# Wang-Ruocheng/QuanONet

Hardware: AMD Instinct MI355X
Metric: train samples/sec (circuit-evals/sec alongside), QuanONet Q=5 Net40-2-20-2 Advection (higher is better)
Workload: dtype f64

## Files before the change

### quanonet_amd/csrc/hea_zyz.hpp

```cpp
#pragma once
#include "hea_device.hpp"
#include "hea_sincos.hpp"

namespace qhea {

constexpr int kRecBytes = 1024;
constexpr int kRecRy = 512;
constexpr int kZCsBytes = 20480;

__host__ __device__ inline long zyz_cs_row(int n, long E) { return E + 2 * n; }
__host__ __device__ inline bool zyz_eligible(int n, long E) {
    return n >= 2 && n <= 5 && (long)(64 >> n) * zyz_cs_row(n, E) * 16 <= kZCsBytes;
}
__host__ __device__ inline int zyz_layer_count(const Runs& r, int n) {
    long L = 0;
    for (int i = 0; i < r.nruns; ++i) L += (long)r.count[i] * ((r.enc[i] + n - 1) / n + r.ld[i]);
    return (int)L;
}

struct AngleSrc {
    const double* x;
    EncDesc enc;
    long m_rows = 0, m_params = 0;
};
// ... 7 lines not shown
    const int si = e < a.enc.seg[0].ncols ? 0 : 1;
    const EncSeg& sg = a.enc.seg[si];
    const int ee = si ? e - a.enc.seg[0].ncols : e;
    const long m = blockIdx.y;
    const double v = sg.in[(b + m * a.m_rows) * sg.width + ee % sg.width];
    const long ep = ee + m * a.m_params;
    return sg.w ? v * sg.w[ep] + sg.b[ep] : v * (MSCALE ? mscale : sg.scale);
}
__device__ __forceinline__ double enc_angle(const AngleSrc& a, int E, long b, int e) { return enc_angle_impl<false>(a, E, b, e, 0.0); }
__device__ __forceinline__ double enc_angle(const AngleSrcM& a, int E, long b, int e) { return enc_angle_impl<true>(a.s, E, b, e, a.scale); }
template <class S>
__device__ __forceinline__ void fill_cs(double2* cs, const S& src, int n, int E, long b0, long B, int ns, int tid, int nthreads,
                                        int row_stride = 0 ) {
    const int row = row_stride ? row_stride : (int)zyz_cs_row(n, E);
    for (int i = tid; i < ns * E; i += nthreads) {
        const int s = i / E, e = i - s * E;
        const long b = (b0 + s < B) ? b0 + s : B - 1;
        double sn, cn;
        fast_sincos(0.5 * enc_angle(src, E, b, e), &sn, &cn);
        cs[s * row + n + e] = make_double2(cn, sn);
    }
}

template <int Q>
__device__ __forceinline__ unsigned lane_sign_mask(int lane) { return ((unsigned)lane << (31 - Q)) & 0x80000000u; }
__device__ __forceinline__ double flip_sign(double v, unsigned mask) {
    return __hiloint2double(__double2hiint(v) ^ (int)mask, __double2loint(v));
}

template <bool DAGGER>
__device__ __forceinline__ void apply_phase(double& re, double& im, const double2& d) {
    const double s = DAGGER ? -d.y : d.y;
    const double nr = d.x * re - s * im;
    im = d.x * im + s * re;
    re = nr;
}
template <int Q, bool DAGGER>
__device__ __forceinline__ void apply_ry(double& re, double& im, const double2& u) {
    const double sv = DAGGER ? -u.y : u.y;
    if constexpr (Q == 4) {
        const auto lo = __builtin_amdgcn_permlane16_swap((unsigned)__double2loint(re), (unsigned)__double2loint(im), false, false);
        const auto hi = __builtin_amdgcn_permlane16_swap((unsigned)__double2hiint(re), (unsigned)__double2hiint(im), false, false);
        const double a = __hiloint2double((int)hi[0], (int)lo[0]), b = __hiloint2double((int)hi[1], (int)lo[1]);
        const double o1 = u.x * a - sv * b, o2 = sv * a + u.x * b;
        const auto l2 = __builtin_amdgcn_permlane16_swap((unsigned)__double2loint(o1), (unsigned)__double2loint(o2), false, false);
        const auto h2 = __builtin_amdgcn_permlane16_swap((unsigned)__double2hiint(o1), (unsigned)__double2hiint(o2), false, false);
        re = __hiloint2double((int)h2[0], (int)l2[0]);
        im = __hiloint2double((int)h2[1], (int)l2[1]);
    } else {
        const double qr = xchg<(1 << Q)>(re), qi = xchg<(1 << Q)>(im);
        re = u.x * re + sv * qr;
        im = u.x * im + sv * qi;
    }
}
template <int N, int Q, bool DAGGER>
__device__ __forceinline__ void apply_enc(double (&re)[1], double (&im)[1], const double2& cs) {
    if constexpr (Q == 4) apply_ry<4, DAGGER>(re[0], im[0], cs);
    else apply_rx<N, Q>(re, im, cs.x, DAGGER ? -cs.y : cs.y);
}

typedef unsigned int u32x4 __attribute__((ext_vector_type(4)));
__device__ __forceinline__ void dma_record(const u32x4& rsrc, unsigned lds_addr, unsigned voff, unsigned soff) {
    asm volatile("s_mov_b32 m0, %0\n\ts_nop 0\n\tbuffer_load_dwordx4 %1, %2, %3 offen lds"
                 :: "s"(lds_addr), "v"(voff), "s"(rsrc), "s"(soff) : "memory", "m0");
}
template <int NREC>
__device__ __forceinline__ void dma_records(const u32x4& rsrc, unsigned lds_addr, unsigned voff, unsigned soff) {
    static_assert(NREC >= 1 && NREC <= 3 && kRecBytes == 1024, "instruction offsets are 12 bits");
    if constexpr (NREC == 1)
        asm volatile("s_mov_b32 m0, %0\n\ts_nop 0\n\tbuffer_load_dwordx4 %1, %2, %3 offen lds"
                     :: "s"(lds_addr), "v"(voff), "s"(rsrc), "s"(soff) : "memory", "m0");
    else if constexpr (NREC == 2)
        asm volatile("s_mov_b32 m0, %0\n\ts_nop 0\n\tbuffer_load_dwordx4 %1, %2, %3 offen lds\n\t"
                     "buffer_load_dwordx4 %1, %2, %3 offen offset:1024 lds"
                     :: "s"(lds_addr), "v"(voff), "s"(rsrc), "s"(soff) : "memory", "m0");
    else
        asm volatile("s_mov_b32 m0, %0\n\ts_nop 0\n\tbuffer_load_dwordx4 %1, %2, %3 offen lds\n\t"
                     "buffer_load_dwordx4 %1, %2, %3 offen offset:1024 lds\n\t"
                     "buffer_load_dwordx4 %1, %2, %3 offen offset:2048 lds"
                     :: "s"(lds_addr), "v"(voff), "s"(rsrc), "s"(soff) : "memory", "m0");
}
template <int CNT>
__device__ __forceinline__ void wait_vmcnt() { asm volatile("s_waitcnt vmcnt(%0)" :: "n"(CNT) : "memory"); }

constexpr int kSlots = 8, kDist = 6;
#ifndef QHEA_ZSIGMA
#define QHEA_ZSIGMA 4
#endif
constexpr int kZSigma = QHEA_ZSIGMA;
constexpr int kAxisRing = 16;
#ifdef QHEA_PROFILE_WAITS
struct ZSync { int psi_prod, lam_prod, ready, abort; int cursor[4]; unsigned long long waited[24]; int next; };
#else
struct ZSync { int psi_prod, lam_prod, ready, abort; int cursor[kZSigma]; int next; };
#endif
constexpr int kRecRingBytes = kSlots * kRecBytes;

template <int N>
struct LayerStream {
    u32x4 rsrc;
    char* ring;
    unsigned lds0;
    unsigned lane16, dgoff;
    unsigned voff[N];
    int L;
    double2 dg;
    double2 ry[N];

    __device__ __forceinline__ void init(const char* table, int bytes, char* ring_wave, int lane, int klow, int nlayers) {
        const unsigned long long base = reinterpret_cast<unsigned long long>(table);
        rsrc = u32x4{(unsigned)base, (unsigned)(base >> 32) & 0xffffu, (unsigned)bytes, 0x00020000u};
        ring = ring_wave;
        lds0 = (unsigned)(unsigned long long)(__attribute__((address_space(3))) char*)ring_wave;
        lane16 = (unsigned)lane * 16u;
        dgoff = (unsigned)klow * 16u;
        L = nlayers;
        static_for<0, N>([&](auto q) {
            constexpr int Q = decltype(q)::value;
            voff[Q] = kRecRy + Q * 32 + (Q == 4 ? 1u : (((unsigned)lane >> Q) & 1u)) * 16u;
        });
    }
    __device__ __forceinline__ void issue(int l) const {
        const int lc = l < 0 ? 0 : (l > L ? L : l);
        dma_record(rsrc, lds0 + (unsigned)(l & (kSlots - 1)) * kRecBytes, lane16, (unsigned)lc * kRecBytes);
    }
    __device__ __forceinline__ char* buf(int l) const { return ring + (l & (kSlots - 1)) * kRecBytes; }
    __device__ __forceinline__ double2 rd_diag(int l) const { return *reinterpret_cast<const double2*>(buf(l) + dgoff); }
    template <int Q>
    __device__ __forceinline__ double2 rd_ry(int l) const { return *reinterpret_cast<const double2*>(buf(l) + voff[Q]); }
    __device__ __forceinline__ void rd_all_ry(int l) { static_for<0, N>([&](auto q) { ry[decltype(q)::value] = rd_ry<decltype(q)::value>(l); }); }

    template <int D>
    __device__ __forceinline__ void prime(int l0) {
#pragma unroll
        for (int i = 0; i < kDist; ++i) issue(l0 + i * D);
        wait_vmcnt<kDist - 1>();
        dg = rd_diag(l0);
        rd_all_ry(l0);
    }
    template <int D>
    __device__ __forceinline__ void begin(int l) {
        issue(l + kDist * D);
        wait_vmcnt<kDist - 1>();
    }
};

template <int N>
__device__ __forceinline__ void zyz_forward(double (&re)[1], double (&im)[1], const Runs& runs, LayerStream<N>& ls,
                                            const double2* __restrict__ csrow, int E, int lane, int klow, int ring_fwd) {
    re[0] = klow == 0 ? 1.0 : 0.0;
    im[0] = 0.0;
    int l = 0, col = 0;
    ls.template prime<1>(0);
    double2 nxt[N];
    auto prefetch = [&](int c) {
        static_for<0, N>([&](auto q) {
            constexpr int Q = decltype(q)::value;
            const int e = c + Q;
            nxt[Q] = csrow[e < E ? e : (E > 0 ? E - 1 : 0)];
        });
    };
    if (E > 0) prefetch(0);
    for (int ri = 0; ri < runs.nruns; ++ri) {
        const int ne = runs.enc[ri], nld = runs.ld[ri];
        for (int rep = 0; rep < runs.count[ri]; ++rep) {
            for (int j0 = 0; j0 < ne; j0 += N) {
                const int m = (ne - j0) < N ? (ne - j0) : N;
                ls.template begin<1>(l);
                apply_phase<false>(re[0], im[0], ls.dg);
                ls.dg = ls.rd_diag(l + 1);
                for_gates_below<N>(m, [&](auto q) {
                    constexpr int Q = decltype(q)::value;
                    apply_enc<N, Q, false>(re, im, nxt[Q]);
                });
                prefetch(col + j0 + m);
                ls.rd_all_ry(l + 1);
                ++l;
            }
            col += ne;
            for (int s = 0; s < nld; ++s) {
                ls.template begin<1>(l);
                apply_phase<false>(re[0], im[0], ls.dg);
                ls.dg = ls.rd_diag(l + 1);
                static_for<0, N>([&](auto q) {
                    constexpr int Q = decltype(q)::value;
                    apply_ry<Q, false>(re[0], im[0], ls.ry[Q]);
                    ls.ry[Q] = ls.template rd_ry<Q>(l + 1);
                });
                re[0] = lane_gather(re[0], ring_fwd);
                im[0] = lane_gather(im[0], ring_fwd);
                ++l;
            }
        }
    }
    apply_phase<false>(re[0], im[0], ls.dg);
}

template <int K> using CtSlot = std::integral_constant<int, K>;
struct RtSlot { int b; };
template <class T> struct is_ct_slot : std::false_type {};
template <int K> struct is_ct_slot<CtSlot<K>> : std::true_type {};
constexpr int kBSlots = 4, kBDist = 2;
constexpr int kPadRecs = 9;
constexpr int kBlockRingBytes = kBSlots * 3 * kRecBytes;

template <int N, int LD, bool SHARED = false>
struct BlockStream {
    static constexpr int RPB = 1 + LD;
    bool loader = true;
    u32x4 rsrc;
    char* ring;
    unsigned lds0, lane16, a_dg;
    unsigned a_ry[N];
    double2 dg[RPB];
    double2 ry[LD][N];
    double2 cs[N];

    __device__ __forceinline__ void init(const char* rec0, int nrec , char* ring_wave, int lane, int klow) {
        const unsigned long long base = reinterpret_cast<unsigned long long>(rec0) - (unsigned long long)kPadRecs * kRecBytes;
        rsrc = u32x4{(unsigned)base, (unsigned)(base >> 32) & 0xffffu, (unsigned)((nrec + 2 * kPadRecs) * kRecBytes), 0x00020000u};
        ring = ring_wave;
        lds0 = (unsigned)(unsigned long long)(__attribute__((address_space(3))) char*)ring_wave;
        lane16 = (unsigned)lane * 16u;
        a_dg = (unsigned)klow * 16u;
        static_for<0, N>([&](auto q) {
            constexpr int Q = decltype(q)::value;
            a_ry[Q] = kRecRy + Q * 32 + (Q == 4 ? 1u : (((unsigned)lane >> Q) & 1u)) * 16u;
        });
    }
    __device__ __forceinline__ void issue(int b) const {
        const unsigned slot = lds0 + (unsigned)(b & (kBSlots - 1)) * (RPB * kRecBytes);
        const unsigned soff = (unsigned)((b * RPB + kPadRecs) * kRecBytes);
        dma_records<RPB>(rsrc, slot, lane16, soff);
    }
    __device__ __forceinline__ const char* slot(int b) const { return ring + (b & (kBSlots - 1)) * (RPB * kRecBytes); }
    template <int D, int K>
    static constexpr int slot_off(CtSlot<K>) { return ((K + D) & (kBSlots - 1)) * (RPB * kRecBytes); }
    template <int D>
    static __device__ __forceinline__ int slot_off(RtSlot s) { return ((s.b + D) & (kBSlots - 1)) * (RPB * kRecBytes); }
    template <int D, class SL>
    __device__ __forceinline__ const char* slot_rel(SL s) const { return ring + slot_off<D>(s); }
    template <int D, class SL>
    __device__ __forceinline__ void ahead_rel(SL s, int b) const {
        if (!SHARED || loader)
            dma_records<RPB>(rsrc, lds0 + (unsigned)slot_off<D>(s), lane16, (unsigned)(((b + D) * RPB + kPadRecs) * kRecBytes));
    }
    __device__ __forceinline__ void landed() const {
        if (!SHARED || loader) wait_vmcnt<(kBDist - 1) * RPB>();
        if constexpr (SHARED) __syncthreads();
    }
    __device__ __forceinline__ void landed_late() const {
        if (!SHARED || loader) wait_vmcnt<kBDist * RPB>();
        if constexpr (SHARED) __syncthreads();
    }
    template <int D>
    __device__ __forceinline__ void ahead(int b) const { if (!SHARED || loader) issue(b + (kBDist + 1) * D); }
    template <int D>
    __device__ __forceinline__ void step(int b) const {
        ahead<D>(b);
        if (!SHARED || loader) wait_vmcnt<kBDist * RPB>();
        if constexpr (SHARED) __syncthreads();
    }
    template <int D>
    __device__ __forceinline__ void prime(int b0, bool drain) const {
        if (!SHARED || loader) {
            if (drain) wait_vmcnt<0>();
        }
        if constexpr (SHARED) { if (drain) __syncthreads(); }
        if (!SHARED || loader) {
#pragma unroll
            for (int i = 0; i <= kBDist; ++i) issue(b0 + i * D);
            wait_vmcnt<kBDist * RPB>();
        }
        if constexpr (SHARED) __syncthreads();
    }
    static __device__ __forceinline__ double2 rd(const char* p, unsigned off) { return *reinterpret_cast<const double2*>(p + off); }
    __device__ __forceinline__ void load_records(const char* sl) {
#pragma unroll
        for (int i = 0; i < RPB; ++i) dg[i] = rd(sl, i * kRecBytes + a_dg);
#pragma unroll
        for (int s = 0; s < LD; ++s)
            static_for<0, N>([&](auto q) { ry[s][decltype(q)::value] = rd(sl, (1 + s) * kRecBytes + a_ry[decltype(q)::value]); });
    }
    __device__ __forceinline__ void load_cs(const double2* __restrict__ csrow, int c0) {
        const double2* p = csrow + c0;
        static_for<0, N>([&](auto q) { cs[decltype(q)::value] = p[decltype(q)::value]; });
    }
};

__host__ __device__ inline int zyz_fast_ld(const Runs& r, int n) {
    if (r.nruns < 1) return 0;
    const int ld = r.ld[0];
    if (ld != 1 && ld != 2) return 0;
    for (int i = 0; i < r.nruns; ++i)
        if (r.ld[i] != ld || r.enc[i] != n || r.count[i] < 1) return 0;
    return ld;
}

template <int N>
struct LayerCoef { double2 dg; double2 g[N]; };

template <int N, int LD, class BS>
__device__ __forceinline__ void zyz_forward_fast(double (&re)[1], double (&im)[1], const Runs& runs, BS& bs,
                                                 const double2* __restrict__ csrow, int E, int lane, int klow, int ring_fwd) {
    re[0] = klow == 0 ? 1.0 : 0.0;
    im[0] = 0.0;
    bs.template prime<1>(0, false);
    int nblocks = 0;
    for (int ri = 0; ri < runs.nruns; ++ri) nblocks += runs.count[ri];
    const double2* cs_b = csrow;
    LayerCoef<N> ce, ca, cb;
    ce.dg = bs.rd(bs.slot(0), bs.a_dg);
    static_for<0, N>([&](auto q) { ce.g[decltype(q)::value] = cs_b[decltype(q)::value]; });
    auto read_layer = [&](LayerCoef<N>& c, const char* sl, int rec) {
        c.dg = bs.rd(sl, rec * kRecBytes + bs.a_dg);
        static_for<0, N>([&](auto q) { c.g[decltype(q)::value] = bs.rd(sl, rec * kRecBytes + bs.a_ry[decltype(q)::value]); });
        __builtin_amdgcn_sched_barrier(0);
    };
    auto read_chunk = [&](const char* nx, int kb) {
        ce.dg = bs.rd(nx, bs.a_dg);
        const double2* cn = cs_b + (kb + 1) * N;
        static_for<0, N>([&](auto q) { ce.g[decltype(q)::value] = cn[decltype(q)::value]; });
        __builtin_amdgcn_sched_barrier(0);
    };
    auto ry_layer = [&](const LayerCoef<N>& c) {
        apply_phase<false>(re[0], im[0], c.dg);
        static_for<0, N>([&](auto q) { apply_ry<decltype(q)::value, false>(re[0], im[0], c.g[decltype(q)::value]); });
        __builtin_amdgcn_sched_barrier(0);
        re[0] = lane_gather(re[0], ring_fwd);
        im[0] = lane_gather(im[0], ring_fwd);
    };
    auto block = [&](auto sl, int b, int kb) {
        const char* cur = bs.template slot_rel<0>(sl);
        const char* nx = bs.template slot_rel<1>(sl);
        read_layer(ca, cur, 1);
        apply_phase<false>(re[0], im[0], ce.dg);
        static_for<0, N>([&](auto q) { apply_enc<N, decltype(q)::value, false>(re, im, ce.g[decltype(q)::value]); });
        if constexpr (LD == 2) {
            read_layer(cb, cur, 2);
            ry_layer(ca);
            bs.template ahead_rel<kBDist + 1>(sl, b);
            __builtin_amdgcn_sched_barrier(0);
            bs.landed_late();
            read_chunk(nx, kb);
            ry_layer(cb);
        } else {
            bs.landed();
            read_chunk(nx, kb);
            ry_layer(ca);
            bs.template ahead_rel<kBDist + 1>(sl, b);
            __builtin_amdgcn_sched_barrier(0);
        }
    };
    int b = 0;
    for (; b + kBSlots <= nblocks; b += kBSlots) {
        block(CtSlot<0>{}, b, 0);
        block(CtSlot<1>{}, b + 1, 1);
        block(CtSlot<2>{}, b + 2, 2);
// ... 23 lines not shown
    }
}
template <int Q>
__device__ __forceinline__ double2 cs32_packed(const double2* chunk ) {
    if constexpr (Q == 4) { const double2 t = chunk[2 * Q]; return make_double2(t.y, t.x); }
    else return chunk[2 * Q + 1];
}

template <bool HALVES>
__device__ __forceinline__ void swap_dup(double x, double& A, double& B) {
    double y;
    asm("" : "=v"(y) : "0"(x));
    const unsigned lo = (unsigned)__double2loint(x), hi = (unsigned)__double2hiint(x);
    const unsigned lo2 = (unsigned)__double2loint(y), hi2 = (unsigned)__double2hiint(y);
    if constexpr (HALVES) {
        const auto l = __builtin_amdgcn_permlane32_swap(lo, lo2, false, false);
        const auto h = __builtin_amdgcn_permlane32_swap(hi, hi2, false, false);
        A = __hiloint2double((int)h[0], (int)l[0]); B = __hiloint2double((int)h[1], (int)l[1]);
    } else {
        const auto l = __builtin_amdgcn_permlane16_swap(lo, lo2, false, false);
        const auto h = __builtin_amdgcn_permlane16_swap(hi, hi2, false, false);
        A = __hiloint2double((int)h[0], (int)l[0]); B = __hiloint2double((int)h[1], (int)l[1]);
    }
}
__device__ __forceinline__ void split_phase(double& x, const double2& d ) {
    double A, B;
    swap_dup<true>(x, A, B);
    x = d.y * A + d.x * B;
}
template <int Q>
__device__ __forceinline__ void split_ry(double& x, const double2& u) {
    if constexpr (Q == 4) {
        double A, B;
        swap_dup<false>(x, A, B);
        x = u.x * A + u.y * B;
    } else {
        const double own = u.x * x;
        x = fma(u.y, xchg<(1 << Q)>(x), own);
    }
}
struct SplitCoef { double2 dg; double t[4]; double2 g4; };
template <int Q>
__device__ __forceinline__ void split_ry_tan(double& x, double t) {
    static_assert(Q < 4, "wire 4 keeps the swap form");
    x = fma(t, xchg<(1 << Q)>(x), x);
}
__device__ __forceinline__ void split_gates(double& x, const LayerCoef<5>& c) {
    static_for<0, 5>([&](auto q) { split_ry<decltype(q)::value>(x, c.g[decltype(q)::value]); });
}
__device__ __forceinline__ void split_gates(double& x, const SplitCoef& c) {
    static_for<0, 4>([&](auto q) { split_ry_tan<decltype(q)::value>(x, c.t[decltype(q)::value]); });
    split_ry<4>(x, c.g4);
}

template <int LD>
struct SplitStream : BlockStream<5, LD, false> {
    using Base = BlockStream<5, LD, false>;
    static constexpr int RPB = 1 + LD;
    unsigned a_cs[5];
    __device__ __forceinline__ void init_split(const char* srec0, int nrec, char* ring_wave, int lane) {
        Base::init(srec0, nrec, ring_wave, lane, lane & 31);
        this->a_dg = (unsigned)(lane & 31) * 24u + (unsigned)(lane >> 5) * 8u;
        static_for<0, 5>([&](auto q) {
            constexpr int Q = decltype(q)::value;
            const unsigned bit = ((unsigned)lane >> Q) & 1u;
            this->a_ry[Q] = Q == 4 ? kSRecRy + 64 + bit * 16u : kSRecRy + Q * 16 + bit * 8u;
            a_cs[Q] = Q * 32 + (Q == 4 ? (1u - bit) : bit) * 16u;
        });
    }
    static __device__ __forceinline__ double2 rd8(const char* p, unsigned off) {
        const double* q = reinterpret_cast<const double*>(p + off);
        return make_double2(q[0], q[1]);
    }
    template <bool DAG = false>
    __device__ __forceinline__ void read_ansatz(SplitCoef& c, const char* sl, int rec, unsigned a_diag) const {
        c.dg = rd8(sl, rec * kRecBytes + a_diag);
        static_for<0, 4>([&](auto q) {
            constexpr int Q = decltype(q)::value;
            c.t[Q] = *reinterpret_cast<const double*>(sl + rec * kRecBytes + (this->a_ry[Q] ^ (DAG ? 8u : 0u)));
        });
        c.g4 = Base::rd(sl, rec * kRecBytes + this->a_ry[4]);
    }
};

constexpr int kSnapBytes = 1024;
template <int LD, bool SNAP = false>
__device__ __forceinline__ double zsplit_forward(SplitStream<LD>& bs, const char* csrow, int nblocks, int lane, int ring_fwd,
                                                 char* snap_base = nullptr, unsigned snap_off = 0) {
    double x = lane == 0 ? 1.0 : 0.0;
    bs.template prime<1>(0, false);
    const char* cs_b = csrow;
    LayerCoef<5> ce;
    SplitCoef ca, cb;
    ce.dg = bs.rd8(bs.slot(0), bs.a_dg);
    static_for<0, 5>([&](auto q) { ce.g[decltype(q)::value] = bs.rd(cs_b, bs.a_cs[decltype(q)::value]); });
    auto read_layer = [&](SplitCoef& c, const char* sl, int rec) {
        bs.read_ansatz(c, sl, rec, bs.a_dg);
        __builtin_amdgcn_sched_barrier(0);
    };
    auto read_chunk = [&](const char* nx, int kb) {
        ce.dg = bs.rd8(nx, bs.a_dg);
        const char* cn = cs_b + (kb + 1) * (5 * 32);
        static_for<0, 5>([&](auto q) { ce.g[decltype(q)::value] = bs.rd(cn, bs.a_cs[decltype(q)::value]); });
        __builtin_amdgcn_sched_barrier(0);
    };
    auto layer = [&](const auto& c, bool ring, int pt) {
        split_phase(x, c.dg);
        split_gates(x, c);
        if constexpr (SNAP) {
            if (ring) {
                typedef __attribute__((address_space(1))) double gdouble;
                *(gdouble*)(snap_base + (size_t)(unsigned)pt * kSnapBytes + snap_off) = x;
            }
        }
        __builtin_amdgcn_sched_barrier(0);
        if (ring) x = lane_gather(x, ring_fwd);
    };
    auto block = [&](auto sl, int b, int kb) {
        const char* cur = bs.template slot_rel<0>(sl);
        const char* nx = bs.template slot_rel<1>(sl);
        read_layer(ca, cur, 1);
        layer(ce, false, 0);
        if constexpr (LD == 2) {
            read_layer(cb, cur, 2);
            layer(ca, true, 2 * b);
            bs.template ahead_rel<kBDist + 1>(sl, b);
            __builtin_amdgcn_sched_barrier(0);
            bs.landed_late();
            read_chunk(nx, kb);
            layer(cb, true, 2 * b + 1);
        } else {
            bs.landed();
            read_chunk(nx, kb);
            layer(ca, true, b);
            bs.template ahead_rel<kBDist + 1>(sl, b);
            __builtin_amdgcn_sched_barrier(0);
        }
    };
    int b = 0;
    for (; b + kBSlots <= nblocks; b += kBSlots) {
        block(CtSlot<0>{}, b, 0);
        block(CtSlot<1>{}, b + 1, 1);
        block(CtSlot<2>{}, b + 2, 2);
        block(CtSlot<3>{}, b + 3, 3);
        cs_b += kBSlots * (5 * 32);
    }
    for (; b < nblocks; ++b) {
        block(RtSlot{b}, b, 0);
        cs_b += 5 * 32;
    }
    split_phase(x, ce.dg);
    return x;
}

struct ZFwdArgs {
    Runs runs; long B; int E; const char* rec; int rec_bytes; int L; AngleSrc src; double off, co;
    const double* diag; int pauli; double* out; double* state_out; const double* bias;
    int fast_ld, nblocks;
    const char* srec;
};
struct MemberStride {
    long rows;
    long params;
    long grad;
    long ws;
};
template <class T>
__host__ __device__ __forceinline__ T* member_ptr(T* p, long bytes) {
    return p ? reinterpret_cast<T*>(reinterpret_cast<typename std::conditional<std::is_const<T>::value, const char, char>::type*>(p) + bytes) : p;
}
struct ZBwdArgs {
    Runs runs; long B; int E; int blk; const char* rec; int rec_bytes; int L; AngleSrc src; double off, co;
    const double* diag; int pauli; const double* g; const double* state_in; const double* y; const double* bias;
// ... 676 lines not shown
            else store_through(&part_w[(long)sub * C::KW + vi], acc3[0]);
        }
    };
    const int LDr = a.fast_ld, nsteps = a.nblocks * LDr;
    const int slot_off = zquad_slot_offset<RING>(LDr, a.nblocks);
    const unsigned snap_lds = (unsigned)(unsigned long long)(__attribute__((address_space(3))) char*)(psi_ring[0]);
    int cur = 0;
    const int vs = sample_slot(lane), ax_slot = vs < 3 * N ? vs : 3 * N - 1;
    const int gx_src1 = sample_slot_lane(vs + 1, lane >> 5) * 4, gx_src2 = sample_slot_lane(vs + 2, lane >> 5) * 4;
    const long bs = wave * C::SPW + (lane >> 5);
    const bool gx_lane = (lane & 1) == 0 && vs < 3 * N && vs % 3 == 0 && bs < a.B;
    double* __restrict__ gx_w = zm_gx(a) + bs * E + vs / 3;
    auto fetch_snap = [&](int t, int sl) {
        asm volatile("s_mov_b32 m0, %0\n\ts_nop 0\n\tbuffer_load_dwordx4 %1, %2, %3 offen sc1 lds"
                     :: "s"(snap_lds + (unsigned)sl * kSnapBytes), "v"((unsigned)lane * 16u), "s"(snap_rsrc),
                        "s"((unsigned)(nsteps - 1 - t) * kSnapBytes) : "memory", "m0");
    };
    auto draw = [&]() {
        int v = 0;
        if (lane == 0) v = __hip_atomic_fetch_add(next, 1, __ATOMIC_RELAXED, __HIP_MEMORY_SCOPE_WORKGROUP);
        return v;
    };
    int mine = __builtin_amdgcn_readfirstlane(draw());
    __hip_atomic_store(&cursor[me], mine, __ATOMIC_RELEASE, __HIP_MEMORY_SCOPE_WORKGROUP);
    int after_v = draw();
    if constexpr (SNAP) {
        if (mine < nsteps) {
#pragma unroll
            for (int i = 0; i < NPROD; ++i) pair_wait_ge(&prod[i], 1, abort_flag, seen_c[i]);
            fetch_snap(mine, 0);
        }
    }
    auto sigma_step = [&](auto chunk_c) {
        constexpr bool CHUNK = decltype(chunk_c)::value;
        const int t = mine;
        const int j = LDr == 2 ? (t >> 1) : t;
        const int sub = a.blk - 1 - t, bl = a.nblocks - 1 - j;
#pragma unroll
        for (int i = 0; i < NPROD; ++i) pair_wait_ge(&prod[i], t + 1, abort_flag, seen_c[i]);
        if constexpr (SNAP) wait_vmcnt<0>();
        const double2* slot = SNAP ? psi_ring[cur] : psi_ring[(t + slot_off) & (RING - 1)];
        const double2 pv = slot[lane];
        double2 qv[N];
        static_for<0, N>([&](auto q) { qv[decltype(q)::value] = slot[lane ^ (1 << decltype(q)::value)]; });
        const double2 lm = lam_ring[(t + slot_off) & (RING - 1)][lane];
        double ax = 0.0;
        if constexpr (CHUNK) ax = axis_ring[(bl & (kAxisRing - 1)) * (3 * N) + ax_slot];
        if (lane == 0) __hip_atomic_store(&cursor[me], after_v, __ATOMIC_RELEASE, __HIP_MEMORY_SCOPE_WORKGROUP);
        mine = __builtin_amdgcn_readfirstlane(after_v);
        after_v = draw();
        if constexpr (SNAP) {
            cur ^= 1;
            if (mine < nsteps) fetch_snap(mine, cur);
        }
        double acc3[C::KW];
        products(acc3, pv, qv, lm);
        if constexpr (CHUNK) {
            sample_butterfly_sum16(acc3, lane);
            const double pr = ax * acc3[0];
            const double g = pr + lane_gather(pr, gx_src1) + lane_gather(pr, gx_src2);
            const double tot = pair_sum<32>(acc3[0]);
            if ((lane & 33) == 0) {
                if constexpr (SNAP) __hip_atomic_fetch_add(&row_lds[sub * C::KW + vs], tot, __ATOMIC_RELAXED, __HIP_MEMORY_SCOPE_WORKGROUP);
                else store_through(&part_w[(long)sub * C::KW + vs], tot);
            }
            if (gx_lane) store_through(&gx_w[bl * N], g);
        } else {
            store_sums(acc3, sub);
        }
    };
    while (mine < nsteps) {
        if (LDr == 1 || (mine & 1)) sigma_step(std::true_type{});
        else sigma_step(std::false_type{});
    }
}

template <int LD, int RING, int NSIG, bool SNAP = false, class A>
__device__ __forceinline__ void zquad_chain(const A& a, int role , int smp, int lane, bool valid, long b,
                                            const char* cs_tables, char* my_ring, double2 (*psi_ring)[64], double2 (*lam_ring)[64],
                                            double2* psi_final, ZQSync* sync, double* axis_ring, char* snap = nullptr) {
    constexpr int N = 5;
    __builtin_amdgcn_s_setprio(3);
    const int E = a.E, k = lane & 31, p = lane >> 5;
    const int ring_fwd = ring_source<N>(lane, false);
    const int ring_rev = ring_source<N>(lane, true);
    const unsigned mask4 = lane_sign_mask<4>(lane);
    SplitStream<LD> ss;
    ss.init_split(zm_srec(a), a.L + 1, my_ring, lane);
    const char* row = cs_tables + (smp * (int)zyz_cs_row(N, E) + N) * 32;
    const int slot_idx = (((smp << 5) | k) << 1) | p;
    int seen[NSIG], safe = 0;
#pragma unroll
    for (int w = 0; w < NSIG; ++w) seen[w] = 0;
    double x;
    if constexpr (SNAP) {
        x = zsplit_forward<LD, true>(ss, row, a.nblocks, lane, ring_fwd, snap, (unsigned)slot_idx * 8u);
        reinterpret_cast<double*>(psi_final)[slot_idx] = x;
        handoff_release();
    } else if (role == 0) {
        if (a.state_in) x = a.state_in[(((b << N) + k) << 1) | p];
        else x = zsplit_forward<LD>(ss, row, a.nblocks, lane, ring_fwd);
        reinterpret_cast<double*>(psi_final)[slot_idx] = x;
        handoff_release();
        if (lane == 0) __hip_atomic_store(&sync->ready[smp], 1, __ATOMIC_RELAXED, __HIP_MEMORY_SCOPE_WORKGROUP);
    }
    if (SNAP || role == 1) {
        int seen_ready = 0;
        if (!SNAP) pair_wait_ge(&sync->ready[smp], 1, &sync->abort, seen_ready);
        const double2 f = psi_final[(smp << 5) | k];
        const double h = ham_weight<N>(k, zm_off(a), zm_co(a), zm_diag(a));
        double v[1] = {h * (f.x * f.x + f.y * f.y)};
        lane_reduce<1, 5>(v, lane);
        const double pred = v[0] + (zm_bias(a) ? zm_bias(a)[0] : 0.0);
        if (zm_out(a) && valid && lane == 0) zm_out(a)[b] = pred;
        double gb = zm_y(a) ? 2.0 * (pred - zm_y(a)[b]) * a.inv_bt : a.g[b];
        if (!valid) gb = 0.0;
        x = gb * h * (p ? f.y : f.x);
    }
    const int nb = a.nblocks;
    double* ring_lane = reinterpret_cast<double*>(role == 0 ? psi_ring : lam_ring) + slot_idx;
    double* ring_pass = ring_lane;
    const int slot_off = zquad_slot_offset<RING>(LD, nb);
    int* prod = role == 0 ? &sync->psi_prod[smp] : &sync->lam_prod[smp];
    int step = 0;
    auto publish_data = [&](auto sl, auto sub) {
        wait_slot_free<NSIG>(sync->cursor, step - RING + 1, &sync->abort, seen, safe);
        if constexpr (LD == 2 && is_ct_slot<decltype(sl)>::value)
            ring_pass[(2 * (kBSlots - 1 - decltype(sl)::value) + decltype(sub)::value) * 128] = x;
        else
            ring_lane[((step + slot_off) & (RING - 1)) * 128] = x;
        ++step;
    };
    auto publish_flag = [&]() {
        handoff_release();
        __hip_atomic_store(prod, step, __ATOMIC_RELAXED, __HIP_MEMORY_SCOPE_WORKGROUP);
    };
    const unsigned a_dgd = (unsigned)k * 24u + (unsigned)(1 - p) * 8u;
    ss.template prime<-1>(nb, true);
    split_phase_dag(x, ss.rd8(ss.slot(nb), a_dgd));
    ss.template step<-1>(nb);
    const char* cs_b = row + (long)(nb - 1) * (N * 32);
    SplitCoef ct, cm;
    LayerCoef<N> c0;
    auto read_layer = [&](SplitCoef& c, const char* sl, int rec) {
        ss.template read_ansatz<true>(c, sl, rec, a_dgd);
        __builtin_amdgcn_sched_barrier(0);
    };
    auto read_chunk = [&](const char* sl, const char* chunk) {
        c0.dg = ss.rd8(sl, a_dgd);
        static_for<0, N>([&](auto q) { c0.g[decltype(q)::value] = ss.rd(chunk, ss.a_cs[decltype(q)::value]); });
        __builtin_amdgcn_sched_barrier(0);
    };
    auto undo_gates = [&](const auto& c) {
        split_gates_dag(x, c, mask4);
        __builtin_amdgcn_sched_barrier(0);
    };
    read_layer(ct, ss.slot(nb - 1), LD);
    static_assert(kAxisRing % kBSlots == 0, "a pass of the unrolled body stays within the axis ring");
    double* axis_lane = axis_ring + lane;
    double* axis_pass = axis_lane;
    typedef double vdouble2 __attribute__((ext_vector_type(2)));
    typedef __attribute__((address_space(3))) const vdouble2 lds_double2;
    unsigned cs_pass[N];
    auto read_chunk_pass = [&](const char* sl, auto k) {
        c0.dg = ss.rd8(sl, a_dgd);
        static_for<0, N>([&](auto q) {
            const vdouble2 v = *(lds_double2*)(unsigned long)(cs_pass[decltype(q)::value] + decltype(k)::value * (N * 32));
            c0.g[decltype(q)::value] = make_double2(v.x, v.y);
        });
        __builtin_amdgcn_sched_barrier(0);
    };
    auto block = [&](auto sl, int bl) {
        const char* cur = ss.template slot_rel<0>(sl);
        const char* nx = ss.template slot_rel<-1>(sl);
        auto chunk_coefs = [&]() {
            if constexpr (is_ct_slot<decltype(sl)>::value) read_chunk_pass(cur, sl);
            else read_chunk(cur, cs_b);
        };
        if (role == 1 && smp == 0 && lane < 3 * N) {
            const double ax = reinterpret_cast<const double*>(cur + kSRecRy)[lane];
            if constexpr (is_ct_slot<decltype(sl)>::value) axis_pass[decltype(sl)::value * (3 * N)] = ax;
            else axis_lane[(bl & (kAxisRing - 1)) * (3 * N)] = ax;
        }
        if constexpr (LD == 2) read_layer(cm, cur, 1);
        else chunk_coefs();
        x = lane_gather(x, ring_rev);
        ss.template ahead_rel<-(kBDist + 1)>(sl, bl);
        __builtin_amdgcn_sched_barrier(0);
        publish_data(sl, std::integral_constant<int, 0>{});
        undo_gates(ct);
        publish_flag();
        if constexpr (LD == 2) {
            chunk_coefs();
            split_phase_dag(x, ct.dg);
            x = lane_gather(x, ring_rev);
            __builtin_amdgcn_sched_barrier(0);
            publish_data(sl, std::integral_constant<int, 1>{});
            undo_gates(cm);
            publish_flag();
            split_phase_dag(x, cm.dg);
        } else {
            split_phase_dag(x, ct.dg);
        }
        ss.landed_late();
        read_layer(ct, nx, LD);
        undo_gates(c0);
        split_phase_dag(x, c0.dg);
    };
    int bl = nb - 1;
    for (; bl >= 0 && (bl & (kBSlots - 1)) != kBSlots - 1; --bl) {
        block(RtSlot{bl}, bl);
        cs_b -= N * 32;
    }
    for (; bl >= kBSlots - 1; bl -= kBSlots) {
        static_for<0, N>([&](auto q) {
            constexpr int Q = decltype(q)::value;
            cs_pass[Q] = (unsigned)(unsigned long long)(__attribute__((address_space(3))) const char*)(cs_b - (kBSlots - 1) * (N * 32)) + ss.a_cs[Q];
            asm("" : "+v"(cs_pass[Q]));
        });
        if constexpr (LD == 2) ring_pass = ring_lane + ((step + slot_off) & (RING - 1) & ~(2 * kBSlots - 1)) * 128;
        axis_pass = axis_lane + (bl & (kAxisRing - 1) & ~(kBSlots - 1)) * (3 * N);
        block(CtSlot<3>{}, bl);
        block(CtSlot<2>{}, bl - 1);
        block(CtSlot<1>{}, bl - 2);
        block(CtSlot<0>{}, bl - 3);
        cs_b -= kBSlots * (N * 32);
    }
}

template <int RING, int NSIG, class A = ZBwdArgs>
__global__ __launch_bounds__(64 * (4 + NSIG)) void bwd_zquad_kernel(A a) {
    constexpr int N = 5;
    using C = Cfg<N>;
    extern __shared__ __attribute__((aligned(16))) char dyn_lds[];
    char* fixed = dyn_lds;
    const int lane = threadIdx.x & 63;
    const int wv = __builtin_amdgcn_readfirstlane((int)(threadIdx.x >> 6));
    const int tid = (int)threadIdx.x;
    char* rec_ring = fixed;
    double2 (*psi_ring)[64] = reinterpret_cast<double2 (*)[64]>(fixed + 4 * kBlockRingBytes);
    double2 (*lam_ring)[64] = reinterpret_cast<double2 (*)[64]>(fixed + 4 * kBlockRingBytes + RING * 1024);
    double2* psi_final = reinterpret_cast<double2*>(fixed + 4 * kBlockRingBytes + 2 * RING * 1024);
    ZQSync& sync = *reinterpret_cast<ZQSync*>(fixed + 4 * kBlockRingBytes + 2 * RING * 1024 + 1024);
    static_assert(sizeof(ZQSync) <= 256, "reserved");
    double* axis_ring = reinterpret_cast<double*>(fixed + 4 * kBlockRingBytes + 2 * RING * 1024 + 1024 + 256);
    char* cs_tables = dyn_lds + zquad_fixed_lds(RING);
    const long wave = blockIdx.x;
    const int E = a.E;
    if (tid == 0) {
        sync.psi_prod[0] = sync.psi_prod[1] = sync.lam_prod[0] = sync.lam_prod[1] = 0;
        sync.ready[0] = sync.ready[1] = 0; sync.abort = 0;
        for (int w = 0; w < NSIG; ++w) sync.cursor[w] = 0;
        sync.next = 0;
    }
    fill_cs_split(reinterpret_cast<double4*>(cs_tables), zm_src(a), E, wave * C::SPW, a.B, C::SPW, tid, 64 * (4 + NSIG));
    __syncthreads();

    if (wv < 4) {
        const int role = wv >> 1, smp = wv & 1;
        const long b_raw = wave * C::SPW + smp;
        const bool valid = b_raw < a.B;
        const long b = valid ? b_raw : a.B - 1;
        char* my_ring = rec_ring + wv * kBlockRingBytes;
        if (a.fast_ld == 2) zquad_chain<2, RING, NSIG>(a, role, smp, lane, valid, b, cs_tables, my_ring, psi_ring, lam_ring, psi_final, &sync, axis_ring);
        else zquad_chain<1, RING, NSIG>(a, role, smp, lane, valid, b, cs_tables, my_ring, psi_ring, lam_ring, psi_final, &sync, axis_ring);
    } else {
        zsigma_walk<RING, 4>(a, lane, wv - 4, wave, psi_ring, lam_ring, axis_ring, &sync.psi_prod[0], &sync.abort, sync.cursor, &sync.next);
    }
    report_abort(&sync.abort, a.status, lane);
}

constexpr int kZSnapRing = 8;
__host__ __device__ constexpr size_t zsnap_fixed_lds(int ring) {
    return 2 * (size_t)kBlockRingBytes + (size_t)ring * 1024 + 1024 + 256 + (size_t)kAxisRing * 15 * sizeof(double) +
           (size_t)kZSigma * 2 * kSnapBytes;
}
template <int RING, class A = ZBwdArgs>
__global__ __launch_bounds__(64 * (4 + 2 * kZSigma)) __attribute__((amdgpu_waves_per_eu(4, 4))) void bwd_zsnap_kernel(A a) {
    constexpr int N = 5;
    using C = Cfg<N>;
    extern __shared__ __attribute__((aligned(16))) char dyn_lds[];
    const int lane = threadIdx.x & 63;
    const int wv = __builtin_amdgcn_readfirstlane((int)(threadIdx.x >> 6));
    const int tid = (int)threadIdx.x;
    const int grp = wv < 4 ? (wv >> 1) : (wv - 4) / kZSigma;
    char* fixed = dyn_lds + grp * (int)zsnap_fixed_lds(RING);
    char* rec_ring = fixed;
    double2 (*lam_ring)[64] = reinterpret_cast<double2 (*)[64]>(fixed + 2 * kBlockRingBytes);
    double2* psi_final = reinterpret_cast<double2*>(fixed + 2 * kBlockRingBytes + RING * 1024);
    ZQSync& sync = *reinterpret_cast<ZQSync*>(fixed + 2 * kBlockRingBytes + RING * 1024 + 1024);
    static_assert(sizeof(ZQSync) <= 256, "reserved");
    double* axis_ring = reinterpret_cast<double*>(fixed + 2 * kBlockRingBytes + RING * 1024 + 1024 + 256);
    char* snap_bufs = fixed + 2 * kBlockRingBytes + RING * 1024 + 1024 + 256 + kAxisRing * 15 * sizeof(double);
    char* lds_tables = dyn_lds + 2 * (int)zsnap_fixed_lds(RING);
    const int E = a.E;
    const int cs_bytes = (int)(C::SPW * zyz_cs_row(N, E) * 32);
    double* row_lds = reinterpret_cast<double*>(lds_tables + 2 * cs_bytes);
    const long wave = (long)blockIdx.x * 2 + grp;
    const int nsteps = a.nblocks * a.fast_ld;
    char* snap = a.snap + wave * (long)nsteps * kSnapBytes;
    if (tid < 2) {
        ZQSync& s = *reinterpret_cast<ZQSync*>(dyn_lds + tid * (int)zsnap_fixed_lds(RING) + 2 * kBlockRingBytes + RING * 1024 + 1024);
        s.psi_prod[0] = s.psi_prod[1] = s.lam_prod[0] = s.lam_prod[1] = 0;
        s.ready[0] = s.ready[1] = 0; s.abort = 0;
        for (int w = 0; w < kZSigma; ++w) s.cursor[w] = 0;
        s.next = 0;
    }
    for (int i = tid; i < a.blk * C::KW; i += 64 * (4 + 2 * kZSigma)) row_lds[i] = 0.0;
    fill_cs_split(reinterpret_cast<double4*>(lds_tables), a.src, E, (long)blockIdx.x * 2 * C::SPW, a.B, 2 * C::SPW, tid, 64 * (4 + 2 * kZSigma));
    __syncthreads();

    if (wv < 4) {
        const int smp = wv & 1;
        const long b_raw = wave * C::SPW + smp;
        const bool valid = b_raw < a.B;
        const long b = valid ? b_raw : a.B - 1;
        char* my_ring = rec_ring + smp * kBlockRingBytes;
        char* cs_tables = lds_tables + grp * cs_bytes;
        char* snap_u = uniform_ptr(snap);
        if (a.fast_ld == 2) zquad_chain<2, RING, kZSigma, true>(a, 1, smp, lane, valid, b, cs_tables, my_ring, lam_ring, lam_ring, psi_final, &sync, axis_ring, snap_u);
        else zquad_chain<1, RING, kZSigma, true>(a, 1, smp, lane, valid, b, cs_tables, my_ring, lam_ring, lam_ring, psi_final, &sync, axis_ring, snap_u);
    } else {
        const int me = (wv - 4) % kZSigma;
        const unsigned long long base = reinterpret_cast<unsigned long long>(uniform_ptr(snap));
        const u32x4 rsrc{(unsigned)base, (unsigned)(base >> 32) & 0xffffu, (unsigned)nsteps * kSnapBytes, 0x00020000u};
        double2 (*buf)[64] = reinterpret_cast<double2 (*)[64]>(snap_bufs + me * 2 * kSnapBytes);
        zsigma_walk<RING, 2, true>(a, lane, me, wave, buf, lam_ring, axis_ring, &sync.lam_prod[0], &sync.abort, sync.cursor, &sync.next,
                                   rsrc, row_lds);
    }
    report_abort(&sync.abort, a.status, lane);
    __syncthreads();
    double* __restrict__ row = zm_part(a) + (long)blockIdx.x * a.blk * C::KW;
    for (int i = tid; i < a.blk * C::KW; i += 64 * (4 + 2 * kZSigma)) store_through(&row[i], row_lds[i]);
}

constexpr int kZPWaves = 4;
__host__ __device__ inline long zp_cs_row(int n, long E) { return E + n; }
__host__ __device__ inline size_t zp_cs_bytes(int n, long E, int rows) { return ((size_t)rows * zp_cs_row(n, E) + n) * sizeof(double2); }

template <int Q>
__device__ __forceinline__ void ry_inv_with_inner(double& pr, double& pi, double& lr, double& li, const double2& u, int lane,
                                                  double& X, double& Y, double& Z) {
    const unsigned m = lane_sign_mask<Q>(lane);
    if constexpr (Q == 4) {
        const double qr = xchg<16>(pr), qi = xchg<16>(pi);
        X = lr * qi - li * qr;
        Y = flip_sign(-(lr * qr) - li * qi, m);
        Z = flip_sign(lr * pi - li * pr, m);
        apply_ry<4, true>(pr, pi, u);
        apply_ry<4, true>(lr, li, u);
    } else {
        const double qr = xchg<(1 << Q)>(pr), qi = xchg<(1 << Q)>(pi);
        X = lr * qi - li * qr;
        Y = flip_sign(-(lr * qr) - li * qi, m);
        Z = flip_sign(lr * pi - li * pr, m);
        pr = u.x * pr - u.y * qr;
        pi = u.x * pi - u.y * qi;
        apply_ry<Q, true>(lr, li, u);
    }
}
template <int N, int Q>
__device__ __forceinline__ void enc_inv_with_inner(double (&pr)[1], double (&pi)[1], double (&lr)[1], double (&li)[1],
                                                   const double2& cs, int lane, double& G) {
    if constexpr (Q == 4) {
        const double qr = xchg<16>(pr[0]), qi = xchg<16>(pi[0]);
        G = flip_sign(-(lr[0] * qr) - li[0] * qi, lane_sign_mask<Q>(lane));
        apply_ry<4, true>(pr[0], pi[0], cs);
        apply_ry<4, true>(lr[0], li[0], cs);
    } else {
        const double qr = xchg<(1 << Q)>(pr[0]), qi = xchg<(1 << Q)>(pi[0]);
        G = lr[0] * qi - li[0] * qr;
        const double nr = cs.x * pr[0] - cs.y * qi;
        pi[0] = cs.x * pi[0] + cs.y * qr;
        pr[0] = nr;
        apply_rx<N, Q>(lr, li, cs.x, -cs.y);
    }
}

template <int N, int LD, class A>
__device__ __forceinline__ void zpacked_body(const A& a, int wib, int lane, int klow, bool valid, long b, long wave,
                                             const double2* cs, char* wg_ring, double* comb ) {
    using C = Cfg<N>;
    const int E = a.E;
    const int ring_fwd = ring_source<N>(lane, false);
    const int ring_rev = ring_source<N>(lane, true);
    const double2* csrow = cs + (wib * C::SPW + (lane >> C::LB)) * (int)zp_cs_row(N, E) + N;
    BlockStream<N, LD, true> bs;
    bs.init(zm_rec(a), a.L + 1, wg_ring, lane, klow);
    bs.loader = wib == 0;

    double pr[1], pi[1], lr[1], li[1];
    if (a.state_in) {
        const double2 s0 = reinterpret_cast<const double2*>(a.state_in)[(b << N) + klow];
        pr[0] = s0.x; pi[0] = s0.y;
    } else {
        zyz_forward_fast<N, LD>(pr, pi, a.runs, bs, csrow, E, lane, klow, ring_fwd);
    }
    {
        double fr[1] = {pr[0]}, fi[1] = {pi[0]};
        basis_change<N, false>(fr, fi, zm_pauli(a), lane);
        const double h = ham_weight<N>(klow, zm_off(a), zm_co(a), zm_diag(a));
        double v[1] = {h * (fr[0] * fr[0] + fi[0] * fi[0])};
        lane_reduce<1, C::LB>(v, lane);
        const double pred = v[0] + (zm_bias(a) ? zm_bias(a)[0] : 0.0);
        if (zm_out(a) && valid && klow == 0) zm_out(a)[b] = pred;
        double gb = zm_y(a) ? 2.0 * (pred - zm_y(a)[b]) * a.inv_bt : a.g[b];
        if (!valid) gb = 0.0;
        lr[0] = gb * h * fr[0]; li[0] = gb * h * fi[0];
        basis_change<N, true>(lr, li, zm_pauli(a), lane);
    }

    const int nb = a.nblocks;
    bs.template prime<-1>(nb, true);
    {
// ... 160 lines not shown
```

Baseline: 14.34 million.

## Prime record stream before LDS setup and prefetch reverse-pass records during forward tail

```diff
diff --git a/quanonet_amd/csrc/hea_zyz.hpp b/quanonet_amd/csrc/hea_zyz.hpp
--- a/quanonet_amd/csrc/hea_zyz.hpp
+++ b/quanonet_amd/csrc/hea_zyz.hpp
@@ -113,6 +113,14 @@
 }
 template <int CNT>
 __device__ __forceinline__ void wait_vmcnt() { asm volatile("s_waitcnt vmcnt(%0)" :: "n"(CNT) : "memory"); }
+
+#ifdef QHEA_CHAIN_STAMPS
+#define QHEA_CHAIN_STAMP(i) do { if (threadIdx.x == 0 && blockIdx.x == gridDim.x / 2) { \
+        extern __shared__ __attribute__((aligned(16))) char qhea_stamp_lds[]; \
+        reinterpret_cast<volatile unsigned long long*>(qhea_stamp_lds + kChainStampOff)[i] = __builtin_amdgcn_s_memtime(); } } while (0)
+#else
+#define QHEA_CHAIN_STAMP(i) do {} while (0)
+#endif
 
 constexpr int kSlots = 8, kDist = 6;
 #ifndef QHEA_ZSIGMA
@@ -234,6 +242,7 @@
 constexpr int kBSlots = 4, kBDist = 2;
 constexpr int kPadRecs = 9;
 constexpr int kBlockRingBytes = kBSlots * 3 * kRecBytes;
+constexpr int kChainStampOff = 2 * kBlockRingBytes + 8 * 1024 + 1024 + 128;
 
 template <int N, int LD, bool SHARED = false>
 struct BlockStream {
@@ -299,12 +308,17 @@
         }
         if constexpr (SHARED) { if (drain) __syncthreads(); }
         if (!SHARED || loader) {
-#pragma unroll
-            for (int i = 0; i <= kBDist; ++i) issue(b0 + i * D);
-            wait_vmcnt<kBDist * RPB>();
+            prime_issue<D>(b0);
+            prime_wait();
         }
         if constexpr (SHARED) __syncthreads();
     }
+    template <int D>
+    __device__ __forceinline__ void prime_issue(int b0) const {
+#pragma unroll
+        for (int i = 0; i <= kBDist; ++i) issue(b0 + i * D);
+    }
+    __device__ __forceinline__ void prime_wait() const { wait_vmcnt<kBDist * RPB>(); }
     static __device__ __forceinline__ double2 rd(const char* p, unsigned off) { return *reinterpret_cast<const double2*>(p + off); }
     __device__ __forceinline__ void load_records(const char* sl) {
 #pragma unroll
@@ -494,13 +508,19 @@
         c.g4 = Base::rd(sl, rec * kRecBytes + this->a_ry[4]);
     }
 };
+__device__ __forceinline__ void split_prime_issue(int ld, const char* srec0, int nrec, char* ring_wave, int lane) {
+    if (ld == 2) { SplitStream<2> s; s.init_split(srec0, nrec, ring_wave, lane); s.template prime_issue<1>(0); }
+    else { SplitStream<1> s; s.init_split(srec0, nrec, ring_wave, lane); s.template prime_issue<1>(0); }
+}
 
 constexpr int kSnapBytes = 1024;
-template <int LD, bool SNAP = false>
+template <int LD, bool SNAP = false, bool PRIMED = false>
 __device__ __forceinline__ double zsplit_forward(SplitStream<LD>& bs, const char* csrow, int nblocks, int lane, int ring_fwd,
                                                  char* snap_base = nullptr, unsigned snap_off = 0) {
     double x = lane == 0 ? 1.0 : 0.0;
-    bs.template prime<1>(0, false);
+    if constexpr (PRIMED) bs.prime_wait();
+    else bs.template prime<1>(0, false);
+    if constexpr (SNAP) QHEA_CHAIN_STAMP(2);
     const char* cs_b = csrow;
     LayerCoef<5> ce;
     SplitCoef ca, cb;
@@ -1343,6 +1363,7 @@
     constexpr int N = 5;
     __builtin_amdgcn_s_setprio(3);
     const int E = a.E, k = lane & 31, p = lane >> 5;
+    const int nb = a.nblocks;
     const int ring_fwd = ring_source<N>(lane, false);
     const int ring_rev = ring_source<N>(lane, true);
     const unsigned mask4 = lane_sign_mask<4>(lane);
@@ -1354,13 +1375,21 @@
 #pragma unroll
     for (int w = 0; w < NSIG; ++w) seen[w] = 0;
     double x;
+    const bool resident = SNAP || (role == 0 && !a.state_in);
+    auto fetch_turn = [&]() {
+        ss.issue(nb - 2);
+        ss.issue(nb - 3);
+    };
     if constexpr (SNAP) {
-        x = zsplit_forward<LD, true>(ss, row, a.nblocks, lane, ring_fwd, snap, (unsigned)slot_idx * 8u);
+        x = zsplit_forward<LD, true, true>(ss, row, nb, lane, ring_fwd, snap, (unsigned)slot_idx * 8u);
+        QHEA_CHAIN_STAMP(3);
+        if (resident) fetch_turn();
         reinterpret_cast<double*>(psi_final)[slot_idx] = x;
         handoff_release();
     } else if (role == 0) {
         if (a.state_in) x = a.state_in[(((b << N) + k) << 1) | p];
-        else x = zsplit_forward<LD>(ss, row, a.nblocks, lane, ring_fwd);
+        else x = zsplit_forward<LD, false, true>(ss, row, nb, lane, ring_fwd);
+        if (resident) fetch_turn();
         reinterpret_cast<double*>(psi_final)[slot_idx] = x;
         handoff_release();
         if (lane == 0) __hip_atomic_store(&sync->ready[smp], 1, __ATOMIC_RELAXED, __HIP_MEMORY_SCOPE_WORKGROUP);
@@ -1377,8 +1406,8 @@
         double gb = zm_y(a) ? 2.0 * (pred - zm_y(a)[b]) * a.inv_bt : a.g[b];
         if (!valid) gb = 0.0;
         x = gb * h * (p ? f.y : f.x);
-    }
-    const int nb = a.nblocks;
+        if constexpr (SNAP) QHEA_CHAIN_STAMP(4);
+    }
     double* ring_lane = reinterpret_cast<double*>(role == 0 ? psi_ring : lam_ring) + slot_idx;
     double* ring_pass = ring_lane;
     const int slot_off = zquad_slot_offset<RING>(LD, nb);
@@ -1395,11 +1424,14 @@
     auto publish_flag = [&]() {
         handoff_release();
         __hip_atomic_store(prod, step, __ATOMIC_RELAXED, __HIP_MEMORY_SCOPE_WORKGROUP);
+#ifdef QHEA_CHAIN_STAMPS
+        if (SNAP && step == 1) QHEA_CHAIN_STAMP(5);
+#endif
     };
     const unsigned a_dgd = (unsigned)k * 24u + (unsigned)(1 - p) * 8u;
-    ss.template prime<-1>(nb, true);
+    if (!resident) ss.template prime<-1>(nb, true);
     split_phase_dag(x, ss.rd8(ss.slot(nb), a_dgd));
-    ss.template step<-1>(nb);
+    if (!resident) ss.template step<-1>(nb);
     const char* cs_b = row + (long)(nb - 1) * (N * 32);
     SplitCoef ct, cm;
     LayerCoef<N> c0;
@@ -1417,6 +1449,7 @@
         __builtin_amdgcn_sched_barrier(0);
     };
     read_layer(ct, ss.slot(nb - 1), LD);
+    if (resident) wait_vmcnt<0>();
     static_assert(kAxisRing % kBSlots == 0, "a pass of the unrolled body stays within the axis ring");
     double* axis_lane = axis_ring + lane;
     double* axis_pass = axis_lane;
@@ -1487,6 +1520,7 @@
         block(CtSlot<0>{}, bl - 3);
         cs_b -= kBSlots * (N * 32);
     }
+    if constexpr (SNAP) QHEA_CHAIN_STAMP(6);
 }
 
 template <int RING, int NSIG, class A = ZBwdArgs>
@@ -1508,6 +1542,12 @@
     char* cs_tables = dyn_lds + zquad_fixed_lds(RING);
     const long wave = blockIdx.x;
     const int E = a.E;
+    const int role = wv >> 1, smp = wv & 1;
+    const long b_raw = wave * C::SPW + smp;
+    const bool valid = b_raw < a.B;
+    const long b = valid ? b_raw : a.B - 1;
+    char* my_ring = rec_ring + wv * kBlockRingBytes;
+    if (wv < 2 && !a.state_in) split_prime_issue(a.fast_ld, zm_srec(a), a.L + 1, my_ring, lane);
     if (tid == 0) {
         sync.psi_prod[0] = sync.psi_prod[1] = sync.lam_prod[0] = sync.lam_prod[1] = 0;
         sync.ready[0] = sync.ready[1] = 0; sync.abort = 0;
@@ -1518,11 +1558,6 @@
     __syncthreads();
 
     if (wv < 4) {
-        const int role = wv >> 1, smp = wv & 1;
-        const long b_raw = wave * C::SPW + smp;
-        const bool valid = b_raw < a.B;
-        const long b = valid ? b_raw : a.B - 1;
-        char* my_ring = rec_ring + wv * kBlockRingBytes;
         if (a.fast_ld == 2) zquad_chain<2, RING, NSIG>(a, role, smp, lane, valid, b, cs_tables, my_ring, psi_ring, lam_ring, psi_final, &sync, axis_ring);
         else zquad_chain<1, RING, NSIG>(a, role, smp, lane, valid, b, cs_tables, my_ring, psi_ring, lam_ring, psi_final, &sync, axis_ring);
     } else {
@@ -1544,6 +1579,7 @@
     const int lane = threadIdx.x & 63;
     const int wv = __builtin_amdgcn_readfirstlane((int)(threadIdx.x >> 6));
     const int tid = (int)threadIdx.x;
+    QHEA_CHAIN_STAMP(0);
     const int grp = wv < 4 ? (wv >> 1) : (wv - 4) / kZSigma;
     char* fixed = dyn_lds + grp * (int)zsnap_fixed_lds(RING);
     char* rec_ring = fixed;
@@ -1560,6 +1596,12 @@
     const long wave = (long)blockIdx.x * 2 + grp;
     const int nsteps = a.nblocks * a.fast_ld;
     char* snap = a.snap + wave * (long)nsteps * kSnapBytes;
+    const int smp = wv & 1;
+    const long b_raw = wave * C::SPW + smp;
+    const bool valid = b_raw < a.B;
+    const long b = valid ? b_raw : a.B - 1;
+    char* my_ring = rec_ring + smp * kBlockRingBytes;
+    if (wv < 4) split_prime_issue(a.fast_ld, zm_srec(a), a.L + 1, my_ring, lane);
     if (tid < 2) {
         ZQSync& s = *reinterpret_cast<ZQSync*>(dyn_lds + tid * (int)zsnap_fixed_lds(RING) + 2 * kBlockRingBytes + RING * 1024 + 1024);
         s.psi_prod[0] = s.psi_prod[1] = s.lam_prod[0] = s.lam_prod[1] = 0;
@@ -1570,13 +1612,9 @@
     for (int i = tid; i < a.blk * C::KW; i += 64 * (4 + 2 * kZSigma)) row_lds[i] = 0.0;
     fill_cs_split(reinterpret_cast<double4*>(lds_tables), a.src, E, (long)blockIdx.x * 2 * C::SPW, a.B, 2 * C::SPW, tid, 64 * (4 + 2 * kZSigma));
     __syncthreads();
+    QHEA_CHAIN_STAMP(1);
 
     if (wv < 4) {
-        const int smp = wv & 1;
-        const long b_raw = wave * C::SPW + smp;
-        const bool valid = b_raw < a.B;
-        const long b = valid ? b_raw : a.B - 1;
-        char* my_ring = rec_ring + smp * kBlockRingBytes;
         char* cs_tables = lds_tables + grp * cs_bytes;
         char* snap_u = uniform_ptr(snap);
         if (a.fast_ld == 2) zquad_chain<2, RING, kZSigma, true>(a, 1, smp, lane, valid, b, cs_tables, my_ring, lam_ring, lam_ring, psi_final, &sync, axis_ring, snap_u);
@@ -1591,6 +1629,16 @@
     }
     report_abort(&sync.abort, a.status, lane);
     __syncthreads();
+#ifdef QHEA_CHAIN_STAMPS
+    if (threadIdx.x == 0 && blockIdx.x == gridDim.x / 2) {
+        static_assert(kChainStampOff == 2 * kBlockRingBytes + RING * 1024 + 1024 + 128 && sizeof(ZQSync) <= 128, "behind group 0's ZQSync");
+        unsigned long long t[8];
+        for (int i = 0; i < 7; ++i) t[i] = reinterpret_cast<volatile unsigned long long*>(dyn_lds + kChainStampOff)[i];
+        t[7] = __builtin_amdgcn_s_memtime();
+        printf("chain stamps: fill %llu | start %llu | forward %llu | turn %llu | to first publication %llu | reverse %llu | tail %llu | total %llu clk\n",
+               t[1] - t[0], t[2] - t[1], t[3] - t[2], t[4] - t[3], t[5] - t[4], t[6] - t[5], t[7] - t[6], t[7] - t[0]);
+    }
+#endif
     double* __restrict__ row = zm_part(a) + (long)blockIdx.x * a.blk * C::KW;
     for (int i = tid; i < a.blk * C::KW; i += 64 * (4 + 2 * kZSigma)) store_through(&row[i], row_lds[i]);
 }
```

Measured after the change: 14.21 million. About the same (-0.9%).
